# ywyue/AGILE3D

Measured on AMD Instinct MI355X. Metric: scenes/s (80k-voxel, 10 clicks), higher is better.
Workload: dtype f32; 1 GPU; batch of 16 synthetic 79736-voxel scenes, 10 clicks each (5 objects x 2), scene build + forward_backbone + 1 forward_mask per scene, fp32, eval; voxels=79736, queries=20, parallelism=scene-sharded x1 (no data-path collective), global_batch=16, steps_in_flight_per_gpu=4

## Files before the change

### agile3d_amd/csrc/decoder.hip

```cpp
#include "common.h"
#include <algorithm>
#include <type_traits>
#include <vector>

namespace a3d {

typedef float f32x4 __attribute__((ext_vector_type(4)));
#define A3D_GLOBAL __attribute__((address_space(1)))
template <typename T>
__device__ __forceinline__ T gld(const T* p) { return *(const T A3D_GLOBAL*)p; }
template <typename T>
__device__ __forceinline__ void gst(T* p, T v) { *(T A3D_GLOBAL*)p = v; }
__device__ __forceinline__ f32x4 gld4(const float* p) { return *(const f32x4 A3D_GLOBAL*)p; }
__device__ __forceinline__ void gst4(float* p, f32x4 v) { *(f32x4 A3D_GLOBAL*)p = v; }
__device__ __forceinline__ bool block_any(int pred, int* slot) {
  if (threadIdx.x == 0) *slot = 0;
  __syncthreads();
  if (pred) *slot = 1;
  __syncthreads();
  return *(volatile int*)slot != 0;
}
template <typename T>
__device__ __forceinline__ T gld_agent(const T* p) {
  return __hip_atomic_load((const T A3D_GLOBAL*)p, __ATOMIC_RELAXED, __HIP_MEMORY_SCOPE_AGENT);
// ... 6 lines not shown
constexpr int H = 8;
constexpr int DH = 16;
constexpr float kLnEps = 1e-5f;
constexpr float kNegBig = -1e30f;
constexpr int kC2SChunk = 128;
constexpr int kPartStride = 18;

__device__ __forceinline__ float rows_max(float x) {
  auto a = __builtin_amdgcn_permlane16_swap(__float_as_uint(x), __float_as_uint(x), false, false);
  x = fmaxf(__uint_as_float(a[0]), __uint_as_float(a[1]));
  auto b = __builtin_amdgcn_permlane32_swap(__float_as_uint(x), __float_as_uint(x), false, false);
  return fmaxf(__uint_as_float(b[0]), __uint_as_float(b[1]));
}
__device__ __forceinline__ float rows_sum(float x) {
  auto a = __builtin_amdgcn_permlane16_swap(__float_as_uint(x), __float_as_uint(x), false, false);
  x = __uint_as_float(a[0]) + __uint_as_float(a[1]);
  auto b = __builtin_amdgcn_permlane32_swap(__float_as_uint(x), __float_as_uint(x), false, false);
  return __uint_as_float(b[0]) + __uint_as_float(b[1]);
}
__device__ __forceinline__ float fast_exp(float x) { return __builtin_amdgcn_exp2f(x * 1.4426950408889634f); }
constexpr float kLog2e = 1.4426950408889634f;
constexpr float kPointScoreScale = 0.25f * kLog2e;
__device__ __forceinline__ float exp2_fast(float x) { return __builtin_amdgcn_exp2f(x); }

__global__ void __launch_bounds__(256) k_minmax_partial(const float* __restrict__ xyz, int n, float* part) {
  __shared__ float s[6][256];
  float mn[3] = {3.4e38f, 3.4e38f, 3.4e38f}, mx[3] = {-3.4e38f, -3.4e38f, -3.4e38f};
  for (int i = blockIdx.x * 256 + threadIdx.x; i < n; i += gridDim.x * 256) {
#pragma unroll
    for (int a = 0; a < 3; ++a) {
      const float v = xyz[3 * (size_t)i + a];
      mn[a] = fminf(mn[a], v);
      mx[a] = fmaxf(mx[a], v);
    }
  }
#pragma unroll
  for (int a = 0; a < 3; ++a) {
    s[a][threadIdx.x] = mn[a];
    s[3 + a][threadIdx.x] = mx[a];
  }
  __syncthreads();
  for (int o = 128; o > 0; o >>= 1) {
    if (threadIdx.x < o) {
#pragma unroll
      for (int a = 0; a < 3; ++a) {
        s[a][threadIdx.x] = fminf(s[a][threadIdx.x], s[a][threadIdx.x + o]);
// ... 315 lines not shown
    }
#pragma unroll
    for (int t = 0; t < 4; ++t) pq[2 + 4 * g + t] = acc[qt][t];
  }
}

template <int QT>
__global__ void __launch_bounds__(512) k_c2s_attn(const float* __restrict__ Kc, const float* __restrict__ V,
                                                  int n, const float* qproj, const int* qobj,
                                                  const unsigned char* labels, const int* counts,
                                                  float* part, int qp_total) {
  c2s_attn_body<QT>(Kc, V, n, qproj, qobj, labels, counts, part, qp_total, (int)blockIdx.y * (QT * 16), QT, (int)blockIdx.x,
                    (int)gridDim.x);
}
template <int QT>
__global__ void __launch_bounds__(512) k_c2s_attn_b(const DecSampleDev* __restrict__ samples) {
  const DecSampleDev& sm = samples[blockIdx.y];
  const int nchunk = (sm.n + kC2SChunk - 1) / kC2SChunk;
  if ((int)blockIdx.x >= nchunk) return;
  c2s_attn_body<QT>(sm.k0, sm.v0, sm.n, sm.qproj, sm.qobj, nullptr, nullptr, sm.part, sm.qp, 0, min(sm.nqt, QT), (int)blockIdx.x, nchunk);
}


template <int QT>
__global__ void __launch_bounds__(512) k_kv_c2s(const DecSampleDev* __restrict__ samples, int ns, int layer,
                                                const float* __restrict__ Wk, const float* __restrict__ Wv,
                                                const float* __restrict__ bk, const float* __restrict__ bv) {
  extern __shared__ __attribute__((aligned(16))) char smem[];
  constexpr int QP = QT * 16;
  constexpr int HW = QT <= 2 ? 4 : 2, WPG = H / HW, SPW = 8 / WPG;
  constexpr bool SWZ = QT == 4;
  constexpr int LDQ = SWZ ? 128 : 132;
  const DecSampleDev& sm = sample_of_wg(samples, ns);
  const int lb = blockIdx.x - sm.wg_begin, nwg = sm.wg_end - sm.wg_begin;
  const int n = sm.n, ngroups = (n + 15) / 16, qp_total = QP;
  const float* __restrict__ X = layer_input(sm, layer);
  const float* __restrict__ Pe = sm.posenc;
  const float* qproj = sm.qproj;
  const int* qobj = sm.qobj;
  const unsigned char* labels = layer > 0 ? sm.labels : nullptr;
  const int* counts = layer > 0 ? sm.counts + (size_t)(layer - 1) * (A3D_MAX_QUERIES + 1) : nullptr;
  float* part = sm.part;
  f32x4* Wkl = (f32x4*)smem;
  f32x4* Wvl = Wkl + 8 * 8 * 64;
  float* qp_l = (float*)(Wvl + 8 * 8 * 64);
  float* bk_l = qp_l + QP * LDQ;
  float* bv_l = bk_l + D;
  const int lane = threadIdx.x & 63, wave = threadIdx.x >> 6;
  const int g = lane >> 4, j = lane & 15;
  const int slot = lb * SPW + wave / WPG, nslots = nwg * SPW;
  f32x4 xs[8], pe[8];
  unsigned lab_nx = 0u;
// ... 11 lines not shown
      f32x4 t8[8];
#pragma unroll
      for (int u = 0; u < 8; ++u) {
        const int e = base + u * 512;
        if (e < TOT) t8[u] = e < TOT / 2 ? ((const f32x4*)Wk)[e] : ((const f32x4*)Wv)[e - TOT / 2];
      }
#pragma unroll
      for (int u = 0; u < 8; ++u)
        if (base + u * 512 < TOT) Wkl[base + u * 512] = t8[u];
    }
  }
  for (int e = threadIdx.x; e < QP * 32; e += 512) {
    const int r = e >> 5, c = e & 31;
    *(f32x4*)(qp_l + r * LDQ + (SWZ ? (c ^ (r & 15)) : c) * 4) = gld4(qproj + (size_t)r * D + c * 4);
  }
  if (!SWZ && threadIdx.x < D) {
    bk_l[threadIdx.x] = bk[threadIdx.x];
    bv_l[threadIdx.x] = bv[threadIdx.x];
  }
  int obj[QT];
  bool qmask[QT];
#pragma unroll
  for (int qt = 0; qt < QT; ++qt) {
    obj[qt] = gld(qobj + qt * 16 + j);
    qmask[qt] = labels != nullptr && obj[qt] >= 0 && gld(counts + obj[qt]) > 0;
  }
  __syncthreads();
  const int h0 = (wave % WPG) * HW;
  f32x4 bkr[HW];
  float bvr[HW];
#pragma unroll
  for (int hl = 0; hl < HW; ++hl) {
    bkr[hl] = (f32x4){0.f, 0.f, 0.f, 0.f};
    bvr[hl] = 0.f;
    if constexpr (SWZ) {
      bkr[hl] = *(const f32x4*)(bk + 16 * (h0 + hl) + 4 * g);
      bvr[hl] = bv[16 * (h0 + hl) + j];
    }
  }
  float m[HW][QT], l[HW][QT];
  f32x4 acc[HW][QT];
#pragma unroll
  for (int hl = 0; hl < HW; ++hl)
#pragma unroll
    for (int qt = 0; qt < QT; ++qt) {
      m[hl][qt] = kNegBig;
      l[hl][qt] = 0.f;
      acc[hl][qt] = (f32x4){0.f, 0.f, 0.f, 0.f};
    }
// ... 20 lines not shown
          const int i2 = S * HW + hl + 1, S2 = i2 / HW, hl2 = i2 % HW;
          f32x4 nk = wk, nv = wv;
          if (i2 < 8 * HW) {
            nk = Wkl[(S2 * 8 + h0 + hl2) * 64 + lane];
            nv = Wvl[(S2 * 8 + h0 + hl2) * 64 + lane];
          }
          __builtin_amdgcn_sched_barrier(0);
#pragma unroll
          for (int t = 0; t < 4; ++t) {
            kf[hl] = __builtin_amdgcn_mfma_f32_16x16x4f32(wk[t], xp[t], kf[hl], 0, 0, 0);
            vv[hl] = __builtin_amdgcn_mfma_f32_16x16x4f32(xs[S][t], wv[t], vv[hl], 0, 0, 0);
          }
          __builtin_amdgcn_sched_barrier(0);
          wk = nk;
          wv = nv;
        }
        xs[S] = gld4(X + nrow * D + 16 * S + 4 * g);
        pe[S] = gld4(Pe + nrow * D + 16 * S + 4 * g);
        __builtin_amdgcn_sched_barrier(0);
      }
    }
    auto qfrag = [&](int qt, int h) {
      const int c = 4 * h + g;
      return *(const f32x4*)(qp_l + (qt * 16 + j) * LDQ + (SWZ ? (c ^ j) : c) * 4);
    };
    f32x4 qf_n = qfrag(0, h0);
    f32x4 mb[QT];
#pragma unroll
    for (int qt = 0; qt < QT; ++qt)
#pragma unroll
      for (int t = 0; t < 4; ++t) {
        const int pr = p0 + 4 * g + t;
        const int lab = (int)((lab4 >> (8 * t)) & 0xffu);
        const bool blocked = pr >= n || (qmask[qt] && lab != obj[qt]);
        mb[qt][t] = blocked ? kNegBig : 0.f;
      }
#pragma unroll
    for (int hl = 0; hl < HW; ++hl) {
      const int h = h0 + hl;
#pragma unroll
      for (int qt = 0; qt < QT; ++qt) {
        const f32x4 qf = qf_n;
        {
          const int i2 = hl * QT + qt + 1;
          if (i2 < HW * QT) qf_n = qfrag(i2 % QT, h0 + i2 / QT);
        }
        f32x4 sc4 = mb[qt];
#pragma unroll
        for (int t = 0; t < 4; ++t) sc4 = __builtin_amdgcn_mfma_f32_16x16x4f32(kf[hl][t], qf[t], sc4, 0, 0, 0);
        float mx = kNegBig;
#pragma unroll
        for (int t = 0; t < 4; ++t) mx = fmaxf(mx, sc4[t]);
        mx = rows_max(mx);
        const float mnew = fmaxf(m[hl][qt], mx);
        const float scl = exp2_fast(m[hl][qt] - mnew);
        m[hl][qt] = mnew;
        f32x4 pw;
        float ps = 0.f;
#pragma unroll
        for (int t = 0; t < 4; ++t) {
          pw[t] = exp2_fast(sc4[t] - mnew);
          ps += pw[t];
        }
        l[hl][qt] = l[hl][qt] * scl + ps;
        acc[hl][qt] *= scl;
#pragma unroll
        for (int t = 0; t < 4; ++t) acc[hl][qt] = __builtin_amdgcn_mfma_f32_16x16x4f32(vv[hl][t], pw[t], acc[hl][qt], 0, 0, 0);
      }
    }
  }
  {
    constexpr int REC = 6 * 64;
    float* red = (float*)smem;
    const int sg = wave / WPG, wl = wave % WPG;
    __syncthreads();
    if (sg > 0) {
#pragma unroll
      for (int hl = 0; hl < HW; ++hl)
#pragma unroll
        for (int qt = 0; qt < QT; ++qt) {
          float* r = red + ((size_t)((sg - 1) * WPG + wl) * (HW * QT) + hl * QT + qt) * REC + lane;
          r[0] = m[hl][qt];
          r[64] = l[hl][qt];
#pragma unroll
          for (int t = 0; t < 4; ++t) r[128 + 64 * t] = acc[hl][qt][t];
        }
    }
    __syncthreads();
    if (sg > 0) return;
#pragma unroll
    for (int hl = 0; hl < HW; ++hl)
#pragma unroll
      for (int qt = 0; qt < QT; ++qt) {
        float mm = m[hl][qt], ll = l[hl][qt];
        f32x4 aa = acc[hl][qt];
#pragma unroll
        for (int o = 1; o < SPW; ++o) {
          const float* r = red + ((size_t)((o - 1) * WPG + wl) * (HW * QT) + hl * QT + qt) * REC + lane;
          const float mo = r[0];
          const float mnew = fmaxf(mm, mo);
          const float sa = exp2_fast(mm - mnew), sb = exp2_fast(mo - mnew);
          mm = mnew;
          ll = ll * sa + r[64] * sb;
#pragma unroll
          for (int t = 0; t < 4; ++t) aa[t] = aa[t] * sa + r[128 + 64 * t] * sb;
        }
        const int h = h0 + hl;
        const float lt = rows_sum(ll);
        float* pq = part + (((size_t)h * qp_total + qt * 16 + j) * nwg + lb) * kPartStride;
        if (g == 0) {
          gst(pq, mm);
          gst(pq + 1, lt);
        }
#pragma unroll
        for (int t = 0; t < 4; ++t) gst(pq + 2 + 4 * g + t, aa[t]);
      }
  }
}
constexpr int kFusedC2SGrid = 256;

__global__ void __launch_bounds__(64) k_c2s_combine(const QuerySample* __restrict__ qs, int cached0) {
  const QuerySample& smp = qs[blockIdx.y];
  const int QP = smp.qp;
  const int q = blockIdx.x / H, h = blockIdx.x % H, lane = threadIdx.x;
  if (q >= smp.meta->nq) return;
  const float* __restrict__ part = smp.part;
  const int nchunk = cached0 ? smp.n_part0 : smp.n_part;
  float* attn = smp.B.attn;
  float m = kNegBig, l = 0.f, o[DH];
#pragma unroll
// ... 468 lines not shown
    if (lane < 16 && p0 + lane < n) {
      float best = Ow[lane * (K + 1)];
      int bi = 0;
      for (int o = 1; o <= K; ++o) {
        const float v = Ow[lane * (K + 1) + o];
        if (v > best) {
          best = v;
          bi = o;
        }
      }
      gst(labels + p0 + lane, (unsigned char)bi);
      atomicAdd(&hist[bi], 1);
    }
    const int rows = min(16, n - p0);
    for (int e = lane; e < rows * (K + 1); e += 64) gst(logits + (size_t)p0 * (K + 1) + e, Ow[e]);
    asm volatile("s_waitcnt lgkmcnt(0)" ::: "memory");
    grp = next;
  }
  __syncthreads();
  for (int e = threadIdx.x; e <= K; e += 512)
    if (hist[e]) atomicAdd(&counts[e], hist[e]);
}

template <int QT, int NW, bool KG = false, bool QC = false>
__global__ void __launch_bounds__(NW * 64) k_s2c_out(const DecSampleDev* __restrict__ samples, int ns, int layer,
                                                 const float* __restrict__ Wq, const float* __restrict__ bq,
                                                 const float* __restrict__ Wo, const float* __restrict__ bo,
                                                 const float* __restrict__ gamma, const float* __restrict__ beta, int nqr_max,
                                                 int Kmax) {
  constexpr int LD = 136, NT = NW * 64;
  constexpr bool PF = NW == 8;
  const DecSampleDev& sm = sample_of_wg(samples, ns);
  const int lb = blockIdx.x - sm.wg_begin, nwg = sm.wg_end - sm.wg_begin;
  const int n = sm.n, ngroups = (n + 15) / 16, nq = sm.nq, n_fg = sm.n_fg, K = sm.K;
  const float* __restrict__ X = layer_input(sm, layer);
  const float* __restrict__ Pe = sm.posenc;
  float* __restrict__ Y = (layer & 1) ? sm.bufD : sm.bufC;
  float* logits = sm.logits + (size_t)layer * n * (K + 1);
  unsigned char* labels = sm.labels;
  int* counts = sm.counts + (size_t)layer * (A3D_MAX_QUERIES + 1);
  const int LT = nqr_max + 4;
  extern __shared__ __attribute__((aligned(16))) char smem[];
  f32x4* Wql = (f32x4*)smem;
  f32x4* Wol = Wql + 8 * 8 * 64;
  float* ks_l = (float*)(Wol + 8 * 8 * 64);
  float* vt_l = ks_l + (KG ? 0 : nqr_max * LD);
  float* bq_l = vt_l + D * LT;
  float* bo_l = bq_l + D;
  float* ga_l = bo_l + D;
  float* be_l = ga_l + D;
  float* O_l = be_l + D;
  int* hist = (int*)(O_l + NW * 16 * (Kmax + 1));
// ... 28 lines not shown
  }
  for (int e = threadIdx.x; e < nqr_max * 32; e += NT) {
    const int r = e >> 5, c4 = (e & 31) * 4;
    f32x4 k4 = (f32x4){0.f, 0.f, 0.f, 0.f}, v4 = k4;
    if (r < nq) {
      k4 = gld4(sm.ks + (size_t)r * D + c4);
      v4 = gld4(sm.vs + (size_t)r * D + c4);
    }
    if constexpr (!KG) *(f32x4*)(ks_l + r * LD + c4) = k4;
#pragma unroll
    for (int t = 0; t < 4; ++t) vt_l[(c4 + t) * LT + r] = v4[t];
  }
  for (int e = threadIdx.x; e < D * 4; e += NT) vt_l[(e >> 2) * LT + nqr_max + (e & 3)] = 0.f;
  const int lane = threadIdx.x & 63, wave = threadIdx.x >> 6;
  const int g = lane >> 4, j = lane & 15;
  __syncthreads();
  float* Ow = O_l + wave * 16 * (Kmax + 1);
  const unsigned lds0 = (unsigned)(size_t)smem;
  const unsigned ks_a0 = (unsigned)(size_t)ks_l + (unsigned)(j * LD + 4 * g) * 4u;
  const unsigned vt_a0 = (unsigned)(size_t)vt_l + (unsigned)(j * LT + 4 * g) * 4u;
  auto lds4 = [](unsigned addr) -> f32x4 { return *(const __attribute__((address_space(3))) f32x4*)addr; };
  const int stride = nwg * NW;
  int grp = lb * NW + wave;
  unsigned oidp[QT];
#pragma unroll
  for (int kt = 0; kt < QT; ++kt) {
    oidp[kt] = 0u;
#pragma unroll
    for (int t = 0; t < 4; ++t) {
      const int q = kt * 16 + 4 * g + t;
      unsigned o = 255u;
      if (q < nq) {
        o = 0u;
        for (int oo = 1; oo <= K; ++oo)
          if (q >= qr_l[oo] && q < qr_l[oo + 1]) o = (unsigned)oo;
      }
      oidp[kt] |= o << (8 * t);
    }
  }
  f32x4 nx[8], np[8];
  auto fetch = [&](int gq) {
    const size_t row = (size_t)min(gq * 16 + j, n - 1);
    const float* xr = X + row * D + 4 * g;
    const float* pr = (QC ? sm.q0 : Pe) + row * D + 4 * g;
#pragma unroll
    for (int S = 0; S < 8; ++S) nx[S] = gld4(xr + 16 * S);
#pragma unroll
    for (int S = 0; S < 8; ++S) np[S] = gld4(pr + 16 * S);
  };
  if (PF && grp < ngroups) fetch(grp);
  while (grp < ngroups) {
    if constexpr (!PF) fetch(grp);
    const int p0 = grp * 16;
    const int prow = min(p0 + j, n - 1);
    f32x4 xp[8], y[8];
#pragma unroll
    for (int S = 0; S < 8; ++S) {
      xp[S] = QC ? np[S] : nx[S] + np[S];
      y[S] = *(const f32x4*)(bo_l + 16 * S + 4 * g) + nx[S];
    }
    const int next = grp + stride;
#pragma unroll 1
    for (int h = 0; h < H; h += 2) {
      if (PF && h == 4 && next < ngroups) fetch(next);
      unsigned wq_a = lds0 + (unsigned)(h * 64 + lane) * 16u;
      unsigned wo_a = lds0 + 65536u + (unsigned)(h * 512 + lane) * 16u;
      unsigned ks_a = KG ? 0u : ks_a0 + (unsigned)(h * DH) * 4u;
      unsigned vt_a = vt_a0 + (unsigned)(h * DH * LT) * 4u;
      asm volatile("" : "+v"(wq_a), "+v"(wo_a), "+v"(vt_a));
      if constexpr (!KG) asm volatile("" : "+v"(ks_a));
      const unsigned vt_a1 = vt_a + (unsigned)(DH * LT) * 4u;
      f32x4 qf[2];
      if constexpr (QC) {
        qf[0] = h == 0 ? xp[0] : h == 2 ? xp[2] : h == 4 ? xp[4] : xp[6];
        qf[1] = h == 0 ? xp[1] : h == 2 ? xp[3] : h == 4 ? xp[5] : xp[7];
      } else {
#pragma unroll
      for (int u = 0; u < 2; ++u) qf[u] = *(const f32x4*)(bq_l + 16 * (h + u) + 4 * g);
      }
      f32x4 kfg[2][QT];
      if constexpr (KG) {
#pragma unroll
        for (int kt = 0; kt < QT; ++kt)
#pragma unroll
          for (int u = 0; u < 2; ++u) kfg[u][kt] = gld4(sm.ks + (size_t)min(kt * 16 + j, nq - 1) * D + (h + u) * DH + 4 * g);
      }
      if constexpr (!QC) {
        f32x4 w0 = lds4(wq_a), w1 = lds4(wq_a + 64 * 16);
#pragma unroll
        for (int S = 0; S < 8; ++S) {
          f32x4 n0 = w0, n1 = w1;
          if (S + 1 < 8) {
            n0 = lds4(wq_a + (S + 1) * 512 * 16);
            n1 = lds4(wq_a + ((S + 1) * 512 + 64) * 16);
          }
          __builtin_amdgcn_sched_barrier(0);
#pragma unroll
          for (int t = 0; t < 4; ++t) {
            qf[0] = __builtin_amdgcn_mfma_f32_16x16x4f32(w0[t], xp[S][t], qf[0], 0, 0, 0);
            qf[1] = __builtin_amdgcn_mfma_f32_16x16x4f32(w1[t], xp[S][t], qf[1], 0, 0, 0);
          }
          __builtin_amdgcn_sched_barrier(0);
          w0 = n0;
          w1 = n1;
        }
      }
      f32x4 sc[2][QT];
      float mx[2] = {kNegBig, kNegBig};
      {
        f32x4 kf[2][QT];
#pragma unroll
        for (int kt = 0; kt < QT; ++kt)
#pragma unroll
          for (int u = 0; u < 2; ++u) {
            if constexpr (KG) kf[u][kt] = kfg[u][kt];
            else kf[u][kt] = lds4(ks_a + (kt * 16 * LD + u * DH) * 4);
            sc[u][kt] = *(const f32x4*)(sb_l + kt * 16 + 4 * g);
          }
#pragma unroll
        for (int t = 0; t < 4; ++t)
#pragma unroll
          for (int kt = 0; kt < QT; ++kt)
#pragma unroll
            for (int u = 0; u < 2; ++u) sc[u][kt] = __builtin_amdgcn_mfma_f32_16x16x4f32(kf[u][kt][t], qf[u][t], sc[u][kt], 0, 0, 0);
      }
#pragma unroll
      for (int u = 0; u < 2; ++u)
#pragma unroll
        for (int kt = 0; kt < QT; ++kt)
#pragma unroll
          for (int t = 0; t < 4; ++t) mx[u] = fmaxf(mx[u], sc[u][kt][t]);
      float inv[2];
#pragma unroll
      for (int u = 0; u < 2; ++u) {
        mx[u] = rows_max(mx[u]);
        float sum = 0.f;
#pragma unroll
        for (int kt = 0; kt < QT; ++kt)
#pragma unroll
          for (int t = 0; t < 4; ++t) {
            sc[u][kt][t] = exp2_fast(sc[u][kt][t] - mx[u]);
            sum += sc[u][kt][t];
          }
        sum = rows_sum(sum);
        inv[u] = __builtin_amdgcn_rcpf(sum);
      }
      f32x4 acc[2] = {(f32x4){0.f, 0.f, 0.f, 0.f}, (f32x4){0.f, 0.f, 0.f, 0.f}};
      f32x4 wo0 = lds4(wo_a), wo1 = lds4(wo_a + 64 * 16);
      {
        f32x4 vf[2][QT];
#pragma unroll
        for (int kt = 0; kt < QT; ++kt)
#pragma unroll
          for (int u = 0; u < 2; ++u) vf[u][kt] = lds4((u ? vt_a1 : vt_a) + kt * 64);
#pragma unroll
        for (int kt = 0; kt < QT; ++kt)
#pragma unroll
          for (int t = 0; t < 4; ++t)
#pragma unroll
            for (int u = 0; u < 2; ++u) acc[u] = __builtin_amdgcn_mfma_f32_16x16x4f32(vf[u][kt][t], sc[u][kt][t], acc[u], 0, 0, 0);
      }
#pragma unroll
      for (int u = 0; u < 2; ++u) acc[u] *= inv[u];
#pragma unroll
      for (int i = 0; i < 8; ++i) {
        const int u = i >> 2, ct = 2 * (i & 3);
        f32x4 n0 = wo0, n1 = wo1;
        if (i + 1 < 8) {
          const int u2 = (i + 1) >> 2, ct2 = 2 * ((i + 1) & 3);
          n0 = lds4(wo_a + (u2 * 512 + ct2 * 64) * 16);
          n1 = lds4(wo_a + (u2 * 512 + ct2 * 64 + 64) * 16);
        }
        __builtin_amdgcn_sched_barrier(0);
#pragma unroll
        for (int t = 0; t < 4; ++t) {
          y[ct] = __builtin_amdgcn_mfma_f32_16x16x4f32(wo0[t], acc[u][t], y[ct], 0, 0, 0);
          y[ct + 1] = __builtin_amdgcn_mfma_f32_16x16x4f32(wo1[t], acc[u][t], y[ct + 1], 0, 0, 0);
        }
        __builtin_amdgcn_sched_barrier(0);
        wo0 = n0;
        wo1 = n1;
      }
    }
    float sum = 0.f;
#pragma unroll
    for (int ct = 0; ct < 8; ++ct) sum += y[ct][0] + y[ct][1] + y[ct][2] + y[ct][3];
    sum = rows_sum(sum);
    const float mean = sum * (1.f / D);
    float var = 0.f;
#pragma unroll
    for (int ct = 0; ct < 8; ++ct)
#pragma unroll
      for (int t = 0; t < 4; ++t) {
        const float d = y[ct][t] - mean;
        var += d * d;
      }
    var = rows_sum(var);
    const float rstd = rsqrtf(var * (1.f / D) + kLnEps);
    float* yrow = Y + (size_t)prow * D;
#pragma unroll
    for (int ct = 0; ct < 8; ++ct) {
      const f32x4 ga = *(const f32x4*)(ga_l + 16 * ct + 4 * g);
      const f32x4 be = *(const f32x4*)(be_l + 16 * ct + 4 * g);
#pragma unroll
      for (int t = 0; t < 4; ++t) y[ct][t] = (y[ct][t] - mean) * rstd * ga[t] + be[t];
      if (p0 + j < n) gst4(yrow + 16 * ct + 4 * g, y[ct]);
    }
    f32x4 ef[QT][8];
#pragma unroll
    for (int qt = 0; qt < QT; ++qt) {
      const float* er = sm.E + (size_t)min(qt * 16 + j, nq - 1) * D + 4 * g;
#pragma unroll
      for (int S = 0; S < 8; ++S) ef[qt][S] = gld4(er + 16 * S);
    }
    f32x4 lg[QT], lg2[QT];
#pragma unroll
    for (int qt = 0; qt < QT; ++qt) lg[qt] = lg2[qt] = (f32x4){0.f, 0.f, 0.f, 0.f};
#pragma unroll
    for (int S = 0; S < 8; S += 2)
#pragma unroll
      for (int t = 0; t < 4; ++t)
#pragma unroll
        for (int qt = 0; qt < QT; ++qt) {
          lg[qt] = __builtin_amdgcn_mfma_f32_16x16x4f32(ef[qt][S][t], y[S][t], lg[qt], 0, 0, 0);
          lg2[qt] = __builtin_amdgcn_mfma_f32_16x16x4f32(ef[qt][S + 1][t], y[S + 1][t], lg2[qt], 0, 0, 0);
        }
#pragma unroll
    for (int qt = 0; qt < QT; ++qt) lg[qt] += lg2[qt];
    float best = 0.f;
    int bi = 0;
    for (int o = 0; o <= K; ++o) {
      float mxv = -3.4e38f;
#pragma unroll
      for (int qt = 0; qt < QT; ++qt)
#pragma unroll
        for (int t = 0; t < 4; ++t)
          if (((oidp[qt] >> (8 * t)) & 255u) == (unsigned)o) mxv = fmaxf(mxv, lg[qt][t]);
      mxv = rows_max(mxv);
      if (g == (o & 3)) Ow[j * (K + 1) + o] = mxv;
      if (o == 0 || mxv > best) {
        best = mxv;
        bi = o;
      }
    }
    if (g == 0 && p0 + j < n) {
      gst(labels + p0 + j, (unsigned char)bi);
      atomicAdd(&hist[bi], 1);
    }
    asm volatile("s_waitcnt lgkmcnt(0)" ::: "memory");
    const int rows = min(16, n - p0);
    for (int e = lane; e < rows * (K + 1); e += 64) gst(logits + (size_t)p0 * (K + 1) + e, Ow[e]);
    asm volatile("s_waitcnt lgkmcnt(0)" ::: "memory");
    grp = next;
  }
  __syncthreads();
  for (int e = threadIdx.x; e <= K; e += NT)
    if (hist[e]) atomicAdd(&counts[e], hist[e]);
}

struct QueryLayerW {
  const float *c2s_in_wt, *c2s_in_b, *c2s_out_wt, *c2s_out_b, *c2s_norm_w, *c2s_norm_b;
  const float *c2c_in_wt, *c2c_in_b, *c2c_out_wt, *c2c_out_b, *c2c_norm_w, *c2c_norm_b;
  const float *ffn_w1t, *ffn_b1, *ffn_w2t, *ffn_b2, *ffn_norm_w, *ffn_norm_b;
  const float *s2c_in_wt, *s2c_in_b;
  const float *dn_w, *dn_b, *m_w0t, *m_b0, *m_w2t, *m_b2;
  const float *next_c2s_in_wt, *next_c2s_in_b;
  const float *qpack, *next_qpack, *mpack;
  int dim_ff;
// ... 1178 lines not shown
      A3D_ALLOW_LDS(big_lds, k_q_s2c<2>);
      A3D_ALLOW_LDS(big_lds, k_q_s2c<3>);
      A3D_ALLOW_LDS(big_lds, k_q_s2c<4>);
      A3D_ALLOW_LDS(big_lds, k_out_ln_mask<1>);
      A3D_ALLOW_LDS(big_lds, k_out_ln_mask<2>);
      A3D_ALLOW_LDS(big_lds, k_out_ln_mask<3>);
      A3D_ALLOW_LDS(big_lds, k_out_ln_mask<4>);
      A3D_ALLOW_LDS(big_lds, k_s2c_out<1, 8>);
      A3D_ALLOW_LDS(big_lds, k_s2c_out<2, 8>);
      A3D_ALLOW_LDS(big_lds, k_s2c_out<1, 12>);
      A3D_ALLOW_LDS(big_lds, k_s2c_out<2, 12>);
      A3D_ALLOW_LDS(big_lds, (k_s2c_out<2, 12, true>));
      A3D_ALLOW_LDS(big_lds, (k_s2c_out<2, 8, true>));
      A3D_ALLOW_LDS(big_lds, (k_s2c_out<1, 12, true>));
      A3D_ALLOW_LDS(big_lds, (k_s2c_out<1, 8, true>));
      A3D_ALLOW_LDS(big_lds, (k_q_s2c<1, true>));
      A3D_ALLOW_LDS(big_lds, (k_q_s2c<2, true>));
      A3D_ALLOW_LDS(big_lds, (k_q_s2c<3, true>));
      A3D_ALLOW_LDS(big_lds, (k_q_s2c<4, true>));
      A3D_ALLOW_LDS(big_lds, (k_s2c_out<1, 12, false, true>));
      A3D_ALLOW_LDS(big_lds, (k_s2c_out<2, 12, false, true>));
      A3D_ALLOW_LDS(big_lds, (k_s2c_out<1, 12, true, true>));
      A3D_ALLOW_LDS(big_lds, (k_s2c_out<2, 12, true, true>));
      A3D_ALLOW_LDS(big_lds, k_kv_c2s<1>);
      A3D_ALLOW_LDS(big_lds, k_kv_c2s<2>);
      A3D_ALLOW_LDS(big_lds, k_kv_c2s<3>);
      A3D_ALLOW_LDS(big_lds, k_kv_c2s<4>);
      A3D_ALLOW_LDS(big_lds, k_ln_mask<4>);
    }
  }
  const int n_counts = A3D_MAX_DEC_LAYERS * (A3D_MAX_QUERIES + 1);
  int64_t n_total = 0;
  int Kmax = 0, nq_max = 0;
  for (int si = 0; si < ns; ++si) {
    Prepared& p = P[si];
    n_total += p.n;
    Kmax = p.hm.K > Kmax ? p.hm.K : Kmax;
    nq_max = p.hm.nq > nq_max ? p.hm.nq : nq_max;
  }
  const size_t s2c_lds = (size_t)2 * QP * 132 * 4;
  const size_t qs2c_lds = ((size_t)QP * 132 + (size_t)D * (QP + 4) + D) * 4;
  const size_t fused_lds = (size_t)64 * 1024 + ((size_t)3 * D + QP * 132 + 8 * 16 * (QP + 1) + 8 * 16 * (Kmax + 1)) * 4 +
                           (size_t)(2 * Kmax + 3) * 4;
  for (int si = 0; si < ns; ++si) {
    const size_t lnm_lds = ((size_t)QP * 132 + 4 * 16 * (P[si].L.qp + 1) + 4 * 16 * (P[si].hm.K + 1)) * 4 + (size_t)(P[si].hm.K + 1) * 4;
    if (lnm_lds > 160 * 1024) {
      set_error("a3d_decoder_forward: %d queries x %d objects need %zu bytes of LDS in the mask head", P[si].hm.nq,
                P[si].hm.K, lnm_lds);
      return A3D_ERR_UNSUPPORTED;
    }
  }
  const bool fuse_c2s = fused_c2s() && nblk == 1;
  const bool fuse_s2c = fused_c2s() && nblk == 1;
  const bool fuse_out = fuse_s2c && fused_lds <= 160 * 1024;
  const int nqr_max = (nq_max + 3) & ~3;
  const size_t s2c_rest = ((size_t)D * (nqr_max + 4) + 4 * D + (size_t)8 * 16 * (Kmax + 1) + 2 * Kmax + 3 + QT * 16 + 1) * 4;
  const size_t s2c_keys = (size_t)nqr_max * 136 * 4;
  const size_t staging12 = (size_t)4 * 16 * (Kmax + 1) * 4;
  const bool s2c_kg = (size_t)128 * 1024 + s2c_keys + s2c_rest + staging12 > 160 * 1024;
  const size_t s2c_out_lds = (size_t)128 * 1024 + (s2c_kg ? 0 : s2c_keys) + s2c_rest;
  const size_t s2c_out_lds12 = s2c_out_lds + staging12;
  static int fused_s2c_env = -1;
// ... 31 lines not shown
          rc = a3d_linear(p.feats, D, p.posenc, D, p.n, D, D, LW.c2s_wk_packed, nullptr, LW.c2s_in_b + D, nullptr, 0, 0, K0, D, nullptr, 0, st);
          if (rc) return rc;
          rc = a3d_linear(p.feats, D, nullptr, 0, p.n, D, D, LW.c2s_wv_packed, nullptr, LW.c2s_in_b + 2 * D, nullptr, 0, 0, V0, D, nullptr, 0, st);
          if (rc) return rc;
          rc = a3d_linear(p.feats, D, p.posenc, D, p.n, D, D, LW.s2c_wq_packed, nullptr, LW.s2c_in_b, nullptr, 0, 0,
                          p.kv0 + (size_t)2 * p.n * D, D, nullptr, 0, st);
          if (rc) return rc;
        }
        if (nblk == 1) continue;
        ProfScope ps(st, A3D_PROF_C2S, 0, 0, 0, 0, p.n);
        k_c2s_attn<QT><<<dim3(p.L.nchunk, nblk), 512, 0, st>>>(K0, V0, p.n, p.B.qproj, p.meta->obj, nullptr, nullptr, p.part, p.L.qp);
        A3D_LAUNCH_CHECK();
      }
      if (nblk == 1) {
        int nchunk_max = 0;
        for (int si = 0; si < ns; ++si) nchunk_max = P[si].L.nchunk > nchunk_max ? P[si].L.nchunk : nchunk_max;
        ProfScope ps(st, A3D_PROF_C2S, 0, 0, 0, 0, (int)n_total);
        k_c2s_attn_b<QT><<<dim3(nchunk_max, ns), 512, 0, st>>>(samples_dev);
        A3D_LAUNCH_CHECK();
      }
    } else if (fuse_c2s) {
      ProfScope ps(st, A3D_PROF_C2S, 0, 0, 0, 0, (int)n_total);
      const size_t c2s_lds = (size_t)128 * 1024 + (QT == 4 ? (size_t)QP * 128 * 4 : ((size_t)QP * 132 + 2 * D) * 4);
      k_kv_c2s<QT><<<grid, 512, c2s_lds, st>>>(samples_dev, ns, l, LW.c2s_wk_packed, LW.c2s_wv_packed, LW.c2s_in_b + D,
                                               LW.c2s_in_b + 2 * D);
      A3D_LAUNCH_CHECK();
    } else {
      for (int si = 0; si < ns; ++si) {
        Prepared& p = P[si];
        const float* src = l == 0 ? p.feats : (((l - 1) & 1) ? p.bufD : p.bufC);
        const int* prev_counts = l > 0 ? p.counts + (size_t)(l - 1) * (A3D_MAX_QUERIES + 1) : nullptr;
        rc = a3d_linear(src, D, p.posenc, D, p.n, D, D, LW.c2s_wk_packed, nullptr, LW.c2s_in_b + D, nullptr, 0, 0, p.bufA, D, nullptr, 0, st);
        if (rc) return rc;
        rc = a3d_linear(src, D, nullptr, 0, p.n, D, D, LW.c2s_wv_packed, nullptr, LW.c2s_in_b + 2 * D, nullptr, 0, 0, p.bufB, D, nullptr, 0, st);
        if (rc) return rc;
        ProfScope ps(st, A3D_PROF_C2S, 0, 0, 0, 0, p.n);
        k_c2s_attn<QT><<<dim3(p.L.nchunk, nblk), 512, 0, st>>>(p.bufA, p.bufB, p.n, p.B.qproj, p.meta->obj,
                                                              l > 0 ? p.labels : nullptr, prev_counts, p.part, p.L.qp);
        A3D_LAUNCH_CHECK();
      }
    }
    rc = launch_query_side<QT>(w, l, qs_dev, P[0].L.qp, nblk, ns, nq_max, cached0, st);
    if (rc) return rc;
    if (fuse_all) {
      ProfScope ps(st, A3D_PROF_S2C, 0, 0, 0, 0, (int)n_total);
      if constexpr (QT <= 2) {
        if (qc0 && s2c_kg && s2c_out_lds12 <= 160 * 1024)
          k_s2c_out<QT, 12, true, true><<<grid, 768, s2c_out_lds12, st>>>(samples_dev, ns, l, LW.s2c_wq_packed, LW.s2c_in_b, LW.s2c_wo_packed,
                                                                         LW.s2c_out_b, LW.s2c_norm_w, LW.s2c_norm_b, nqr_max, Kmax);
        else if (qc0 && !s2c_kg && s2c_out_lds12 <= 160 * 1024)
          k_s2c_out<QT, 12, false, true><<<grid, 768, s2c_out_lds12, st>>>(samples_dev, ns, l, LW.s2c_wq_packed, LW.s2c_in_b, LW.s2c_wo_packed,
                                                                          LW.s2c_out_b, LW.s2c_norm_w, LW.s2c_norm_b, nqr_max, Kmax);
        else if (s2c_kg && s2c_out_lds12 <= 160 * 1024)
          k_s2c_out<QT, 12, true><<<grid, 768, s2c_out_lds12, st>>>(samples_dev, ns, l, LW.s2c_wq_packed, LW.s2c_in_b, LW.s2c_wo_packed,
                                                                   LW.s2c_out_b, LW.s2c_norm_w, LW.s2c_norm_b, nqr_max, Kmax);
        else if (s2c_kg)
          k_s2c_out<QT, 8, true><<<grid, 512, s2c_out_lds, st>>>(samples_dev, ns, l, LW.s2c_wq_packed, LW.s2c_in_b, LW.s2c_wo_packed,
                                                                LW.s2c_out_b, LW.s2c_norm_w, LW.s2c_norm_b, nqr_max, Kmax);
        else if (s2c_out_lds12 <= 160 * 1024)
          k_s2c_out<QT, 12><<<grid, 768, s2c_out_lds12, st>>>(samples_dev, ns, l, LW.s2c_wq_packed, LW.s2c_in_b, LW.s2c_wo_packed,
                                                             LW.s2c_out_b, LW.s2c_norm_w, LW.s2c_norm_b, nqr_max, Kmax);
        else
          k_s2c_out<QT, 8><<<grid, 512, s2c_out_lds, st>>>(samples_dev, ns, l, LW.s2c_wq_packed, LW.s2c_in_b, LW.s2c_wo_packed,
                                                          LW.s2c_out_b, LW.s2c_norm_w, LW.s2c_norm_b, nqr_max, Kmax);
      }
      A3D_LAUNCH_CHECK();
      continue;
    }
    if (fuse_s2c) {
      ProfScope ps(st, A3D_PROF_S2C, 0, 0, 0, 0, (int)n_total);
      if (qc0) k_q_s2c<QT, true><<<grid, 512, (size_t)64 * 1024 + qs2c_lds, st>>>(samples_dev, ns, l, LW.s2c_wq_packed, LW.s2c_in_b);
      else k_q_s2c<QT><<<grid, 512, (size_t)64 * 1024 + qs2c_lds, st>>>(samples_dev, ns, l, LW.s2c_wq_packed, LW.s2c_in_b);
      A3D_LAUNCH_CHECK();
    } else {
      for (int si = 0; si < ns; ++si) {
        Prepared& p = P[si];
        const float* src = l == 0 ? p.feats : (((l - 1) & 1) ? p.bufD : p.bufC);
        const float* Qs = p.bufA;
        if (qc0) {
          Qs = p.kv0 + (size_t)2 * p.n * D;
        } else {
          rc = a3d_linear(src, D, p.posenc, D, p.n, D, D, LW.s2c_wq_packed, nullptr, LW.s2c_in_b, nullptr, 0, 0, p.bufA, D, nullptr, 0, st);
          if (rc) return rc;
        }
        ProfScope ps(st, A3D_PROF_S2C, 0, 0, 0, 0, p.n);
        k_s2c_attn_wide<QT><<<(p.n + 127) / 128, 512, s2c_lds, st>>>(Qs, p.n, p.B.ks, p.B.vs, p.hm.nq, nblk, p.bufB);
        A3D_LAUNCH_CHECK();
// ... 383 lines not shown
```

Measured before the change: 636.0 scenes/s.

## Handle leftover query rows with 4x4 MFMA and add lazy softmax rescale

When every scene has 17–20 queries, the second 16-query tile is mostly padding. A leftover variant of the c2s and s2c kernels computes the extra 4 queries with 4x4x1 MFMA and permlane reductions instead of a full 16x16 tile. Separately, the online softmax in k_kv_c2s now rescales only when a ballot sees the max rise by more than a threshold. The last decoder layer also skips writing outputs and labels it will not use. This trades wasted MFMA work for more cross-lane shuffles, and relies on that threshold staying numerically safe.

```diff
diff --git a/agile3d_amd/csrc/decoder.hip b/agile3d_amd/csrc/decoder.hip
--- a/agile3d_amd/csrc/decoder.hip
+++ b/agile3d_amd/csrc/decoder.hip
@@ -52,6 +52,28 @@
 constexpr float kLog2e = 1.4426950408889634f;
 constexpr float kPointScoreScale = 0.25f * kLog2e;
 __device__ __forceinline__ float exp2_fast(float x) { return __builtin_amdgcn_exp2f(x); }
+
+__device__ __forceinline__ f32x4 mfma4(float a, float b, f32x4 c) { return __builtin_amdgcn_mfma_f32_4x4x1f32(a, b, c, 0, 0, 0); }
+__device__ __forceinline__ float rows_sum_scatter(f32x4 s) {
+  auto a = __builtin_amdgcn_permlane32_swap(__float_as_uint(s[0]), __float_as_uint(s[1]), false, false);
+  auto b = __builtin_amdgcn_permlane32_swap(__float_as_uint(s[2]), __float_as_uint(s[3]), false, false);
+  const float r01 = __uint_as_float(a[0]) + __uint_as_float(a[1]);
+  const float r23 = __uint_as_float(b[0]) + __uint_as_float(b[1]);
+  auto c = __builtin_amdgcn_permlane16_swap(__float_as_uint(r01), __float_as_uint(r23), false, false);
+  return __uint_as_float(c[0]) + __uint_as_float(c[1]);
+}
+__device__ __forceinline__ int row_reg(int g) { return ((g & 1) << 1) | (g >> 1); }
+__device__ __forceinline__ float row_bcast(float x, int lane4, int row) {
+  return __int_as_float(__builtin_amdgcn_ds_bpermute(lane4 + 64 * row, __float_as_int(x)));
+}
+__device__ __forceinline__ float quads_max(float x) {
+  x = fmaxf(x, __shfl_xor(x, 4, 64));
+  return fmaxf(x, __shfl_xor(x, 8, 64));
+}
+__device__ __forceinline__ float quads_sum(float x) {
+  x += __shfl_xor(x, 4, 64);
+  return x + __shfl_xor(x, 8, 64);
+}
 
 __global__ void __launch_bounds__(256) k_minmax_partial(const float* __restrict__ xyz, int n, float* part) {
   __shared__ float s[6][256];
@@ -413,12 +435,14 @@
 }
 
 
-template <int QT>
+template <int QT, bool LO = false>
 __global__ void __launch_bounds__(512) k_kv_c2s(const DecSampleDev* __restrict__ samples, int ns, int layer,
                                                 const float* __restrict__ Wk, const float* __restrict__ Wv,
                                                 const float* __restrict__ bk, const float* __restrict__ bv) {
   extern __shared__ __attribute__((aligned(16))) char smem[];
   constexpr int QP = QT * 16;
+  static_assert(!LO || QT == 2, "the leftover-tile build is the two-tile kernel");
+  constexpr float kRefLazy = 8.f;
   constexpr int HW = QT <= 2 ? 4 : 2, WPG = H / HW, SPW = 8 / WPG;
   constexpr bool SWZ = QT == 4;
   constexpr int LDQ = SWZ ? 128 : 132;
@@ -476,9 +500,10 @@
   bool qmask[QT];
 #pragma unroll
   for (int qt = 0; qt < QT; ++qt) {
-    obj[qt] = gld(qobj + qt * 16 + j);
+    obj[qt] = gld(qobj + ((LO && qt == 1) ? 16 + (j & 3) : qt * 16 + j));
     qmask[qt] = labels != nullptr && obj[qt] >= 0 && gld(counts + obj[qt]) > 0;
   }
+  const int lo_pt = (j & 12) + row_reg(g), lo_src = (4 * g + (j & 3)) * 4;
   __syncthreads();
   const int h0 = (wave % WPG) * HW;
   f32x4 bkr[HW];
@@ -545,7 +570,8 @@
     }
     auto qfrag = [&](int qt, int h) {
       const int c = 4 * h + g;
-      return *(const f32x4*)(qp_l + (qt * 16 + j) * LDQ + (SWZ ? (c ^ j) : c) * 4);
+      const int r = (LO && qt == 1) ? 16 + (j & 3) : qt * 16 + j;
+      return *(const f32x4*)(qp_l + r * LDQ + (SWZ ? (c ^ j) : c) * 4);
     };
     f32x4 qf_n = qfrag(0, h0);
     f32x4 mb[QT];
@@ -558,6 +584,12 @@
         const bool blocked = pr >= n || (qmask[qt] && lab != obj[qt]);
         mb[qt][t] = blocked ? kNegBig : 0.f;
       }
+    float mb_lo = 0.f;
+    if constexpr (LO) {
+      const unsigned labw = (unsigned)__shfl((int)lab4, 16 * (lo_pt >> 2), 64);
+      const int lab = (int)((labw >> (8 * (lo_pt & 3))) & 0xffu);
+      mb_lo = (p0 + lo_pt >= n || (qmask[1] && lab != obj[1])) ? kNegBig : 0.f;
+    }
 #pragma unroll
     for (int hl = 0; hl < HW; ++hl) {
       const int h = h0 + hl;
@@ -568,25 +600,43 @@
           const int i2 = hl * QT + qt + 1;
           if (i2 < HW * QT) qf_n = qfrag(i2 % QT, h0 + i2 / QT);
         }
+        if constexpr (LO) {
+          if (qt == 1) {
+            f32x4 s4 = (f32x4){0.f, 0.f, 0.f, 0.f};
+#pragma unroll
+            for (int t = 0; t < 4; ++t) s4 = mfma4(kf[hl][t], qf[t], s4);
+            const float sc1 = rows_sum_scatter(s4) + mb_lo;
+            if (__builtin_amdgcn_ballot_w64(sc1 - m[hl][1] > kRefLazy) != 0) {
+              const float mnew = fmaxf(m[hl][1], rows_max(quads_max(sc1)));
+              const float scl = exp2_fast(m[hl][1] - mnew);
+              m[hl][1] = mnew;
+              l[hl][1] *= scl;
+              acc[hl][1] *= scl;
+            }
+            const float pw1 = exp2_fast(sc1 - m[hl][1]);
+            l[hl][1] += pw1;
+#pragma unroll
+            for (int t = 0; t < 4; ++t) {
+              acc[hl][1] = mfma4(vv[hl][t], row_bcast(pw1, lo_src, row_reg(t)), acc[hl][1]);
+            }
+            continue;
+          }
+        }
         f32x4 sc4 = mb[qt];
 #pragma unroll
         for (int t = 0; t < 4; ++t) sc4 = __builtin_amdgcn_mfma_f32_16x16x4f32(kf[hl][t], qf[t], sc4, 0, 0, 0);
-        float mx = kNegBig;
-#pragma unroll
-        for (int t = 0; t < 4; ++t) mx = fmaxf(mx, sc4[t]);
-        mx = rows_max(mx);
-        const float mnew = fmaxf(m[hl][qt], mx);
-        const float scl = exp2_fast(m[hl][qt] - mnew);
-        m[hl][qt] = mnew;
+        const float mx4 = fmaxf(fmaxf(sc4[0], sc4[1]), fmaxf(sc4[2], sc4[3]));
+        if (__builtin_amdgcn_ballot_w64(mx4 - m[hl][qt] > kRefLazy) != 0) {
+          const float mnew = fmaxf(m[hl][qt], rows_max(mx4));
+          const float scl = exp2_fast(m[hl][qt] - mnew);
+          m[hl][qt] = mnew;
+          l[hl][qt] *= scl;
+          acc[hl][qt] *= scl;
+        }
         f32x4 pw;
-        float ps = 0.f;
-#pragma unroll
-        for (int t = 0; t < 4; ++t) {
-          pw[t] = exp2_fast(sc4[t] - mnew);
-          ps += pw[t];
-        }
-        l[hl][qt] = l[hl][qt] * scl + ps;
-        acc[hl][qt] *= scl;
+#pragma unroll
+        for (int t = 0; t < 4; ++t) pw[t] = exp2_fast(sc4[t] - m[hl][qt]);
+        l[hl][qt] += (pw[0] + pw[1]) + (pw[2] + pw[3]);
 #pragma unroll
         for (int t = 0; t < 4; ++t) acc[hl][qt] = __builtin_amdgcn_mfma_f32_16x16x4f32(vv[hl][t], pw[t], acc[hl][qt], 0, 0, 0);
       }
@@ -629,6 +679,23 @@
           for (int t = 0; t < 4; ++t) aa[t] = aa[t] * sa + r[128 + 64 * t] * sb;
         }
         const int h = h0 + hl;
+        if constexpr (LO) {
+          if (qt == 1) {
+            const float lt = rows_sum(quads_sum(ll));
+            float* pq = part + (((size_t)h * qp_total + 16 + (j & 3)) * nwg + lb) * kPartStride;
+#pragma unroll
+            for (int t = 0; t < 4; ++t) aa[t] = rows_sum(aa[t]);
+            if (g == 0) {
+              if (j < 4) {
+                gst(pq, mm);
+                gst(pq + 1, lt);
+              }
+#pragma unroll
+              for (int t = 0; t < 4; ++t) gst(pq + 2 + (j & 12) + t, aa[t]);
+            }
+            continue;
+          }
+        }
         const float lt = rows_sum(ll);
         float* pq = part + (((size_t)h * qp_total + qt * 16 + j) * nwg + lb) * kPartStride;
         if (g == 0) {
@@ -1143,12 +1210,14 @@
     if (hist[e]) atomicAdd(&counts[e], hist[e]);
 }
 
-template <int QT, int NW, bool KG = false, bool QC = false>
+template <int QT, int NW, bool KG = false, bool QC = false, bool LO = false>
 __global__ void __launch_bounds__(NW * 64) k_s2c_out(const DecSampleDev* __restrict__ samples, int ns, int layer,
                                                  const float* __restrict__ Wq, const float* __restrict__ bq,
                                                  const float* __restrict__ Wo, const float* __restrict__ bo,
                                                  const float* __restrict__ gamma, const float* __restrict__ beta, int nqr_max,
-                                                 int Kmax) {
+                                                 int Kmax, int last) {
+  static_assert(!LO || (QT == 2 && !KG), "the leftover-tile build is the two-tile kernel with the keys in LDS");
+  constexpr int QF = LO ? 1 : QT;
   constexpr int LD = 136, NT = NW * 64;
   constexpr bool PF = NW == 8;
   const DecSampleDev& sm = sample_of_wg(samples, ns);
@@ -1223,9 +1292,9 @@
   auto lds4 = [](unsigned addr) -> f32x4 { return *(const __attribute__((address_space(3))) f32x4*)addr; };
   const int stride = nwg * NW;
   int grp = lb * NW + wave;
-  unsigned oidp[QT];
-#pragma unroll
-  for (int kt = 0; kt < QT; ++kt) {
+  unsigned oidp[QF];
+#pragma unroll
+  for (int kt = 0; kt < QF; ++kt) {
     oidp[kt] = 0u;
 #pragma unroll
     for (int t = 0; t < 4; ++t) {
@@ -1238,6 +1307,19 @@
       }
       oidp[kt] |= o << (8 * t);
     }
+  }
+  float sb_lo = 0.f;
+  unsigned oid_lo = 255u, ks_lo0 = 0u, vt_lo0 = 0u;
+  if constexpr (LO) {
+    const int q = 16 + row_reg(g);
+    sb_lo = q < nq ? 0.f : kNegBig;
+    if (q < nq) {
+      oid_lo = 0u;
+      for (int oo = 1; oo <= K; ++oo)
+        if (q >= qr_l[oo] && q < qr_l[oo + 1]) oid_lo = (unsigned)oo;
+    }
+    ks_lo0 = (unsigned)(size_t)ks_l + (unsigned)((16 + (j & 3)) * LD + 4 * g) * 4u;
+    vt_lo0 = (unsigned)(size_t)vt_l + (unsigned)((4 * g + (j & 3)) * LT + 16) * 4u;
   }
   f32x4 nx[8], np[8];
   auto fetch = [&](int gq) {
@@ -1279,7 +1361,7 @@
 #pragma unroll
       for (int u = 0; u < 2; ++u) qf[u] = *(const f32x4*)(bq_l + 16 * (h + u) + 4 * g);
       }
-      f32x4 kfg[2][QT];
+      f32x4 kfg[2][QF];
       if constexpr (KG) {
 #pragma unroll
         for (int kt = 0; kt < QT; ++kt)
@@ -1306,12 +1388,21 @@
           w1 = n1;
         }
       }
-      f32x4 sc[2][QT];
+      f32x4 sc[2][QF];
       float mx[2] = {kNegBig, kNegBig};
+      float s1[2] = {0.f, 0.f};
       {
-        f32x4 kf[2][QT];
-#pragma unroll
-        for (int kt = 0; kt < QT; ++kt)
+        f32x4 kf[2][QF];
+        f32x4 kl[2], s4[2];
+        if constexpr (LO) {
+#pragma unroll
+          for (int u = 0; u < 2; ++u) {
+            kl[u] = lds4(ks_lo0 + (unsigned)((h + u) * DH) * 4u);
+            s4[u] = (f32x4){0.f, 0.f, 0.f, 0.f};
+          }
+        }
+#pragma unroll
+        for (int kt = 0; kt < QF; ++kt)
 #pragma unroll
           for (int u = 0; u < 2; ++u) {
             if constexpr (KG) kf[u][kt] = kfg[u][kt];
@@ -1319,16 +1410,28 @@
             sc[u][kt] = *(const f32x4*)(sb_l + kt * 16 + 4 * g);
           }
 #pragma unroll
-        for (int t = 0; t < 4; ++t)
-#pragma unroll
-          for (int kt = 0; kt < QT; ++kt)
+        for (int t = 0; t < 4; ++t) {
+#pragma unroll
+          for (int kt = 0; kt < QF; ++kt)
 #pragma unroll
             for (int u = 0; u < 2; ++u) sc[u][kt] = __builtin_amdgcn_mfma_f32_16x16x4f32(kf[u][kt][t], qf[u][t], sc[u][kt], 0, 0, 0);
+          if constexpr (LO) {
+#pragma unroll
+            for (int u = 0; u < 2; ++u) s4[u] = mfma4(kl[u][t], qf[u][t], s4[u]);
+          }
+        }
+        if constexpr (LO) {
+#pragma unroll
+          for (int u = 0; u < 2; ++u) {
+            s1[u] = rows_sum_scatter(s4[u]) + sb_lo;
+            mx[u] = s1[u];
+          }
+        }
       }
 #pragma unroll
       for (int u = 0; u < 2; ++u)
 #pragma unroll
-        for (int kt = 0; kt < QT; ++kt)
+        for (int kt = 0; kt < QF; ++kt)
 #pragma unroll
           for (int t = 0; t < 4; ++t) mx[u] = fmaxf(mx[u], sc[u][kt][t]);
       float inv[2];
@@ -1337,29 +1440,49 @@
         mx[u] = rows_max(mx[u]);
         float sum = 0.f;
 #pragma unroll
-        for (int kt = 0; kt < QT; ++kt)
+        for (int kt = 0; kt < QF; ++kt)
 #pragma unroll
           for (int t = 0; t < 4; ++t) {
             sc[u][kt][t] = exp2_fast(sc[u][kt][t] - mx[u]);
             sum += sc[u][kt][t];
           }
+        if constexpr (LO) {
+          s1[u] = exp2_fast(s1[u] - mx[u]);
+          sum += s1[u];
+        }
         sum = rows_sum(sum);
         inv[u] = __builtin_amdgcn_rcpf(sum);
       }
       f32x4 acc[2] = {(f32x4){0.f, 0.f, 0.f, 0.f}, (f32x4){0.f, 0.f, 0.f, 0.f}};
       f32x4 wo0 = lds4(wo_a), wo1 = lds4(wo_a + 64 * 16);
       {
-        f32x4 vf[2][QT];
-#pragma unroll
-        for (int kt = 0; kt < QT; ++kt)
+        f32x4 vf[2][QF];
+        f32x4 vl[2];
+        float pl[2][4];
+        if constexpr (LO) {
+#pragma unroll
+          for (int u = 0; u < 2; ++u) {
+            vl[u] = lds4(vt_lo0 + (unsigned)((h + u) * DH * LT) * 4u);
+#pragma unroll
+            for (int t = 0; t < 4; ++t) pl[u][t] = row_bcast(s1[u], j * 4, row_reg(t));
+          }
+        }
+#pragma unroll
+        for (int kt = 0; kt < QF; ++kt)
 #pragma unroll
           for (int u = 0; u < 2; ++u) vf[u][kt] = lds4((u ? vt_a1 : vt_a) + kt * 64);
 #pragma unroll
-        for (int kt = 0; kt < QT; ++kt)
+        for (int kt = 0; kt < QF; ++kt)
 #pragma unroll
           for (int t = 0; t < 4; ++t)
 #pragma unroll
             for (int u = 0; u < 2; ++u) acc[u] = __builtin_amdgcn_mfma_f32_16x16x4f32(vf[u][kt][t], sc[u][kt][t], acc[u], 0, 0, 0);
+        if constexpr (LO) {
+#pragma unroll
+          for (int t = 0; t < 4; ++t)
+#pragma unroll
+            for (int u = 0; u < 2; ++u) acc[u] = mfma4(vl[u][t], pl[u][t], acc[u]);
+        }
       }
 #pragma unroll
       for (int u = 0; u < 2; ++u) acc[u] *= inv[u];
@@ -1405,38 +1528,63 @@
       const f32x4 be = *(const f32x4*)(be_l + 16 * ct + 4 * g);
 #pragma unroll
       for (int t = 0; t < 4; ++t) y[ct][t] = (y[ct][t] - mean) * rstd * ga[t] + be[t];
-      if (p0 + j < n) gst4(yrow + 16 * ct + 4 * g, y[ct]);
-    }
-    f32x4 ef[QT][8];
-#pragma unroll
-    for (int qt = 0; qt < QT; ++qt) {
+      if (!last && p0 + j < n) gst4(yrow + 16 * ct + 4 * g, y[ct]);
+    }
+    f32x4 ef[QF][8];
+#pragma unroll
+    for (int qt = 0; qt < QF; ++qt) {
       const float* er = sm.E + (size_t)min(qt * 16 + j, nq - 1) * D + 4 * g;
 #pragma unroll
       for (int S = 0; S < 8; ++S) ef[qt][S] = gld4(er + 16 * S);
     }
-    f32x4 lg[QT], lg2[QT];
-#pragma unroll
-    for (int qt = 0; qt < QT; ++qt) lg[qt] = lg2[qt] = (f32x4){0.f, 0.f, 0.f, 0.f};
-#pragma unroll
-    for (int S = 0; S < 8; S += 2)
-#pragma unroll
-      for (int t = 0; t < 4; ++t)
-#pragma unroll
-        for (int qt = 0; qt < QT; ++qt) {
+    f32x4 lg[QF], lg2[QF];
+#pragma unroll
+    for (int qt = 0; qt < QF; ++qt) lg[qt] = lg2[qt] = (f32x4){0.f, 0.f, 0.f, 0.f};
+    f32x4 ll4 = (f32x4){0.f, 0.f, 0.f, 0.f}, ll4b = ll4, el[2] = {ll4, ll4};
+    const float* erl = nullptr;
+    if constexpr (LO) {
+      erl = sm.E + (size_t)min(16 + (j & 3), nq - 1) * D + 4 * g;
+      el[0] = gld4(erl);
+      el[1] = gld4(erl + 16);
+    }
+#pragma unroll
+    for (int S = 0; S < 8; S += 2) {
+      f32x4 e0 = el[0], e1 = el[1];
+      if constexpr (LO) {
+        if (S + 2 < 8) {
+          el[0] = gld4(erl + 16 * (S + 2));
+          el[1] = gld4(erl + 16 * (S + 3));
+        }
+      }
+#pragma unroll
+      for (int t = 0; t < 4; ++t) {
+#pragma unroll
+        for (int qt = 0; qt < QF; ++qt) {
           lg[qt] = __builtin_amdgcn_mfma_f32_16x16x4f32(ef[qt][S][t], y[S][t], lg[qt], 0, 0, 0);
           lg2[qt] = __builtin_amdgcn_mfma_f32_16x16x4f32(ef[qt][S + 1][t], y[S + 1][t], lg2[qt], 0, 0, 0);
         }
-#pragma unroll
-    for (int qt = 0; qt < QT; ++qt) lg[qt] += lg2[qt];
+        if constexpr (LO) {
+          ll4 = mfma4(e0[t], y[S][t], ll4);
+          ll4b = mfma4(e1[t], y[S + 1][t], ll4b);
+        }
+      }
+    }
+#pragma unroll
+    for (int qt = 0; qt < QF; ++qt) lg[qt] += lg2[qt];
+    float l1 = 0.f;
+    if constexpr (LO) l1 = rows_sum_scatter(ll4 + ll4b);
     float best = 0.f;
     int bi = 0;
     for (int o = 0; o <= K; ++o) {
       float mxv = -3.4e38f;
 #pragma unroll
-      for (int qt = 0; qt < QT; ++qt)
+      for (int qt = 0; qt < QF; ++qt)
 #pragma unroll
         for (int t = 0; t < 4; ++t)
           if (((oidp[qt] >> (8 * t)) & 255u) == (unsigned)o) mxv = fmaxf(mxv, lg[qt][t]);
+      if constexpr (LO) {
+        if (oid_lo == (unsigned)o) mxv = fmaxf(mxv, l1);
+      }
       mxv = rows_max(mxv);
       if (g == (o & 3)) Ow[j * (K + 1) + o] = mxv;
       if (o == 0 || mxv > best) {
@@ -1444,7 +1592,7 @@
         bi = o;
       }
     }
-    if (g == 0 && p0 + j < n) {
+    if (!last && g == 0 && p0 + j < n) {
       gst(labels + p0 + j, (unsigned char)bi);
       atomicAdd(&hist[bi], 1);
     }
@@ -2669,6 +2817,9 @@
       A3D_ALLOW_LDS(big_lds, (k_s2c_out<2, 12, false, true>));
       A3D_ALLOW_LDS(big_lds, (k_s2c_out<1, 12, true, true>));
       A3D_ALLOW_LDS(big_lds, (k_s2c_out<2, 12, true, true>));
+      A3D_ALLOW_LDS(big_lds, (k_s2c_out<2, 12, false, false, true>));
+      A3D_ALLOW_LDS(big_lds, (k_s2c_out<2, 12, false, true, true>));
+      A3D_ALLOW_LDS(big_lds, (k_kv_c2s<2, true>));
       A3D_ALLOW_LDS(big_lds, k_kv_c2s<1>);
       A3D_ALLOW_LDS(big_lds, k_kv_c2s<2>);
       A3D_ALLOW_LDS(big_lds, k_kv_c2s<3>);
@@ -2678,13 +2829,15 @@
   }
   const int n_counts = A3D_MAX_DEC_LAYERS * (A3D_MAX_QUERIES + 1);
   int64_t n_total = 0;
-  int Kmax = 0, nq_max = 0;
+  int Kmax = 0, nq_max = 0, nq_min = A3D_MAX_QUERIES;
   for (int si = 0; si < ns; ++si) {
     Prepared& p = P[si];
     n_total += p.n;
     Kmax = p.hm.K > Kmax ? p.hm.K : Kmax;
     nq_max = p.hm.nq > nq_max ? p.hm.nq : nq_max;
-  }
+    nq_min = p.hm.nq < nq_min ? p.hm.nq : nq_min;
+  }
+  const bool leftover = QT == 2 && nq_min >= 17 && nq_max <= 20;
   const size_t s2c_lds = (size_t)2 * QP * 132 * 4;
   const size_t qs2c_lds = ((size_t)QP * 132 + (size_t)D * (QP + 4) + D) * 4;
   const size_t fused_lds = (size_t)64 * 1024 + ((size_t)3 * D + QP * 132 + 8 * 16 * (QP + 1) + 8 * 16 * (Kmax + 1)) * 4 +
@@ -2762,8 +2915,12 @@
     } else if (fuse_c2s) {
       ProfScope ps(st, A3D_PROF_C2S, 0, 0, 0, 0, (int)n_total);
       const size_t c2s_lds = (size_t)128 * 1024 + (QT == 4 ? (size_t)QP * 128 * 4 : ((size_t)QP * 132 + 2 * D) * 4);
-      k_kv_c2s<QT><<<grid, 512, c2s_lds, st>>>(samples_dev, ns, l, LW.c2s_wk_packed, LW.c2s_wv_packed, LW.c2s_in_b + D,
-                                               LW.c2s_in_b + 2 * D);
+      if (QT == 2 && leftover)
+        k_kv_c2s<2, true><<<grid, 512, c2s_lds, st>>>(samples_dev, ns, l, LW.c2s_wk_packed, LW.c2s_wv_packed, LW.c2s_in_b + D,
+                                                      LW.c2s_in_b + 2 * D);
+      else
+        k_kv_c2s<QT><<<grid, 512, c2s_lds, st>>>(samples_dev, ns, l, LW.c2s_wk_packed, LW.c2s_wv_packed, LW.c2s_in_b + D,
+                                                 LW.c2s_in_b + 2 * D);
       A3D_LAUNCH_CHECK();
     } else {
       for (int si = 0; si < ns; ++si) {
@@ -2784,25 +2941,32 @@
     if (rc) return rc;
     if (fuse_all) {
       ProfScope ps(st, A3D_PROF_S2C, 0, 0, 0, 0, (int)n_total);
+      const int last = l + 1 == w->n_layers;
       if constexpr (QT <= 2) {
-        if (qc0 && s2c_kg && s2c_out_lds12 <= 160 * 1024)
+        if (leftover && qc0 && !s2c_kg && s2c_out_lds12 <= 160 * 1024)
+          k_s2c_out<2, 12, false, true, true><<<grid, 768, s2c_out_lds12, st>>>(samples_dev, ns, l, LW.s2c_wq_packed, LW.s2c_in_b, LW.s2c_wo_packed,
+                                                                               LW.s2c_out_b, LW.s2c_norm_w, LW.s2c_norm_b, nqr_max, Kmax, last);
+        else if (leftover && !qc0 && !s2c_kg && s2c_out_lds12 <= 160 * 1024)
+          k_s2c_out<2, 12, false, false, true><<<grid, 768, s2c_out_lds12, st>>>(samples_dev, ns, l, LW.s2c_wq_packed, LW.s2c_in_b, LW.s2c_wo_packed,
+                                                                                LW.s2c_out_b, LW.s2c_norm_w, LW.s2c_norm_b, nqr_max, Kmax, last);
+        else if (qc0 && s2c_kg && s2c_out_lds12 <= 160 * 1024)
           k_s2c_out<QT, 12, true, true><<<grid, 768, s2c_out_lds12, st>>>(samples_dev, ns, l, LW.s2c_wq_packed, LW.s2c_in_b, LW.s2c_wo_packed,
-                                                                         LW.s2c_out_b, LW.s2c_norm_w, LW.s2c_norm_b, nqr_max, Kmax);
+                                                                         LW.s2c_out_b, LW.s2c_norm_w, LW.s2c_norm_b, nqr_max, Kmax, last);
         else if (qc0 && !s2c_kg && s2c_out_lds12 <= 160 * 1024)
           k_s2c_out<QT, 12, false, true><<<grid, 768, s2c_out_lds12, st>>>(samples_dev, ns, l, LW.s2c_wq_packed, LW.s2c_in_b, LW.s2c_wo_packed,
-                                                                          LW.s2c_out_b, LW.s2c_norm_w, LW.s2c_norm_b, nqr_max, Kmax);
+                                                                          LW.s2c_out_b, LW.s2c_norm_w, LW.s2c_norm_b, nqr_max, Kmax, last);
         else if (s2c_kg && s2c_out_lds12 <= 160 * 1024)
           k_s2c_out<QT, 12, true><<<grid, 768, s2c_out_lds12, st>>>(samples_dev, ns, l, LW.s2c_wq_packed, LW.s2c_in_b, LW.s2c_wo_packed,
-                                                                   LW.s2c_out_b, LW.s2c_norm_w, LW.s2c_norm_b, nqr_max, Kmax);
+                                                                   LW.s2c_out_b, LW.s2c_norm_w, LW.s2c_norm_b, nqr_max, Kmax, last);
         else if (s2c_kg)
           k_s2c_out<QT, 8, true><<<grid, 512, s2c_out_lds, st>>>(samples_dev, ns, l, LW.s2c_wq_packed, LW.s2c_in_b, LW.s2c_wo_packed,
-                                                                LW.s2c_out_b, LW.s2c_norm_w, LW.s2c_norm_b, nqr_max, Kmax);
+                                                                LW.s2c_out_b, LW.s2c_norm_w, LW.s2c_norm_b, nqr_max, Kmax, last);
         else if (s2c_out_lds12 <= 160 * 1024)
           k_s2c_out<QT, 12><<<grid, 768, s2c_out_lds12, st>>>(samples_dev, ns, l, LW.s2c_wq_packed, LW.s2c_in_b, LW.s2c_wo_packed,
-                                                             LW.s2c_out_b, LW.s2c_norm_w, LW.s2c_norm_b, nqr_max, Kmax);
+                                                             LW.s2c_out_b, LW.s2c_norm_w, LW.s2c_norm_b, nqr_max, Kmax, last);
         else
           k_s2c_out<QT, 8><<<grid, 512, s2c_out_lds, st>>>(samples_dev, ns, l, LW.s2c_wq_packed, LW.s2c_in_b, LW.s2c_wo_packed,
-                                                          LW.s2c_out_b, LW.s2c_norm_w, LW.s2c_norm_b, nqr_max, Kmax);
+                                                          LW.s2c_out_b, LW.s2c_norm_w, LW.s2c_norm_b, nqr_max, Kmax, last);
       }
       A3D_LAUNCH_CHECK();
       continue;
```

Measured after the change: 648.3 scenes/s (median of 6 runs). 1.9% higher.
